# facebookresearch/brainmagick

Measured on AMD Instinct MI355X. Metric: segments/s, 208-ch x 360-sample SimpleConv + ClipLoss training step, higher is better.
Workload: dtype f32 (fp32-accurate: operands split into 2 scaled f16 planes, 3 MFMA products, fp32 accumulate; same parity tolerances as exact fp32, see DESIGN.md §2); 1 GPU; cfg2: gwilliams2022-shaped MEG C=208 T=360, F=120 features, 27 subjects, clip_conv SimpleConv (8985590 params) + ClipLoss + Adam; batch_per_gpu=256, global_batch=256, negatives=local, parallelism=dp1, comm=none, rccl_world=1, candidate_gather=none, distinct_batches=8

## Files before the change

### brainmagick_amd/functional.py

```python

import torch

from . import hip_ops as H



ACT_CODES = {"none": H.ACT_NONE, "gelu": H.ACT_GELU, "relu": H.ACT_RELU, "leaky": H.ACT_LEAKY}


def _c(t: torch.Tensor) -> torch.Tensor:
    return t if t.is_contiguous() else t.contiguous()


_arange_cache = {}


def _arange_i32(n: int, device, repeat: int = 1) -> torch.Tensor:
    key = (n, repeat, device.type, device.index)
    t = _arange_cache.get(key)
    if t is None:
        if len(_arange_cache) > 64:
            _arange_cache.clear()
        t = torch.arange(n, dtype=torch.int32, device=device)
        if repeat != 1:
# ... 49 lines not shown
    if ctx.needs_input_grad[1]:
        if pad is None:
            dw = _conv_weight_grads(dy, x, weight, KS, dil, transposed)
        else:
            a, xl = (x, dy) if transposed else (dy, x)
            dw = H.conv_strided_wgrad(a, xl, KS, stride, dil, pad, out=H.grad_destination(weight)).view(weight.shape)
    dx = None
    if ctx.needs_input_grad[0]:
        if pad is not None:
            wp = H.pack_strided_rows_first(weight) if transposed else H.pack_strided_rows_second(weight)
            _, dx, _ = H.conv_strided(dy, wp, Cin, T, KS, stride, dil, pad, not transposed)
        else:
            if transposed:
                M = weight.shape[1]
                wp = H.pack_weights(weight, 1, Cin, M, 1, 0, M, 1, 0, shape=(T, dil))
            else:
                wp = H.pack_conv_dgrad(weight, (T, dil))
            _, dx, _ = H.conv_nn(dy, wp, Cin, KS, dil, res=res, publish_amax=publish_amax)
    return dx, dw


class Conv1dFn(torch.autograd.Function):

    @staticmethod
    def forward(ctx, x, weight, bias, dil: int, act: int, leak: float, transposed_weight: bool, stride: int = 1,
                pad=None):
        x, weight = _c(x), _c(weight)
        geom = (dil, transposed_weight, stride, pad)
        need_pre = act != H.ACT_NONE and any(ctx.needs_input_grad[:3])
        if need_pre and pad is None:
            pre, _, _ = _layer_forward(x, weight, geom, bias=bias, want_pre=True, want_out=False)
            out = H.affine_act_res(pre, None, None, None, act, leak)
        else:
            pre, out, _ = _layer_forward(x, weight, geom, bias=bias, act=act, leak=leak, want_pre=need_pre)
        ctx.save_for_backward(x, weight, pre)
        ctx.cfg = (geom, act, leak, bias is not None)
        return out

    @staticmethod
    def backward(ctx, dout):
        x, weight, pre = ctx.saved_tensors
        geom, act, leak, has_bias = ctx.cfg
        dout = _c(dout)
        dbias = None
        if act != H.ACT_NONE:
            dy, _, _, dbias = H.act_bn_bwd(dout, pre, None, None, None, None, False, act, leak,
                                           want_dbias=has_bias)
        else:
            dy = dout
            if has_bias:
                dbias = H.channel_sum(dy)
        dx, dw = _layer_backward(ctx, dy, x, weight, geom)
        return (dx, dw, dbias) + (None,) * 6


class ConvBNActFn(torch.autograd.Function):

    @staticmethod
    def forward(ctx, x, weight, bias, gamma, beta, running_mean, running_var, num_batches,
                training: bool, dil: int, act: int, leak: float, residual: bool, momentum: float,
                eps: float, stride: int = 1, pad=None, transposed: bool = False):
        x, weight = _c(x), _c(weight)
        geom = (dil, transposed, stride, pad)
        res = x if residual else None
        needs_grad = any(ctx.needs_input_grad[:5])
        if training:
            pre, _, stats = _layer_forward(x, weight, geom, bias=bias, want_pre=True, want_out=False, want_stats=True)
            mean, invstd, scale, shift = H.bn_finalize(stats, pre.shape[0] * pre.shape[2], gamma, beta, running_mean,
                                                       running_var, num_batches, momentum, eps)
            out = H.affine_act_res(pre, scale, shift, res, act, leak)
        else:
            mean, invstd, scale, shift = H.bn_eval_affine(gamma, beta, running_mean, running_var, eps)
            pre, out, _ = _layer_forward(x, weight, geom, res=res, bias=bias, scale=scale, shift=shift, act=act,
                                         leak=leak, want_pre=needs_grad)
        ctx.save_for_backward(x, weight, pre, scale, shift, mean, invstd)
        ctx.cfg = (geom, training, act, leak, residual, bias is not None)
        return out

    @staticmethod
    def backward(ctx, dout):
        x, weight, pre, scale, shift, mean, invstd = ctx.saved_tensors
        geom, training, act, leak, residual, has_bias = ctx.cfg
        dout = _c(dout)
        dy, dgamma, dbeta, dbias = H.act_bn_bwd(dout, pre, scale, shift, mean, invstd, training, act,
                                                leak, want_affine_grads=True, want_dbias=has_bias)
        dx, dw = _layer_backward(ctx, dy, x, weight, geom, res=dout if residual else None, publish_amax=False)
        return (dx, dw, dbias, dgamma, dbeta) + (None,) * 13


class GLUConvFn(torch.autograd.Function):

    @staticmethod
    def forward(ctx, x, weight, bias):
        x, weight = _c(x), _c(weight)
        M, Cin, KS = weight.shape
        u, _, _ = H.conv_nn(x, H.pack_conv_fwd(weight, (x.shape[2], 1)), M, KS, 1, bias=bias, want_pre=True,
                            want_out=False)
        out = H.glu_fwd(u)
        ctx.save_for_backward(x, weight, u)
        ctx.has_bias = bias is not None
        return out

    @staticmethod
    def backward(ctx, dout):
        x, weight, u = ctx.saved_tensors
        M, Cin, KS = weight.shape
# ... 404 lines not shown
```

### brainmagick_amd/hip_ops.py

```python
import ctypes
import typing as tp

import numpy as np
import torch

from ._lib import lib, check, BmHipError

ACT_NONE, ACT_GELU, ACT_RELU, ACT_LEAKY = 0, 1, 2, 3
BKC = 16

import os as _os
DEFAULT_COMPUTE_DTYPE = "f16x2"
COMPUTE_DTYPES = ("f32", "f32x3", "f16x2")
_compute_dtype = _os.environ.get("BM_COMPUTE_DTYPE", DEFAULT_COMPUTE_DTYPE)
if _compute_dtype not in COMPUTE_DTYPES:
    raise ValueError(f"BM_COMPUTE_DTYPE must be one of {COMPUTE_DTYPES}, got {_compute_dtype!r}")


def set_compute_dtype(name: str):
    global _compute_dtype
    if name not in COMPUTE_DTYPES:
        raise ValueError(f"compute dtype must be one of {COMPUTE_DTYPES}, got {name!r}")
    _compute_dtype = name

# ... 208 lines not shown
        e["used"] = _weights_epoch
        if e["stamp"] != (_weights_epoch, src._version):
            self.refresh()
        return e["dst"]

    def refresh(self):
        global pack_launches
        stale = [k for k, e in self.entries.items()
                 if e["used"] < _weights_epoch - self.KEEP or e["src"].data_ptr() != e["ptr"]]
        for k in stale:
            del self.entries[k]
        if stale:
            self.table = None
        ents = list(self.entries.values())
        if not ents:
            return
        if self.table is None:
            nb = lib().bm_pack_h2_job_bytes()
            host = ctypes.create_string_buffer(nb * len(ents))
            block0 = 0
            for i, e in enumerate(ents):
                n = lib().bm_pack_h2_job_fill(ctypes.c_void_p(ctypes.addressof(host) + i * nb), _p(e["src"]),
                                              _p(e["dst"]), *e["geom"], None, block0)
                if n < 0:
                    raise BmHipError("bm_pack_h2_job_fill: bad arguments %r" % (e["geom"],))
                block0 += n
            self.table = torch.frombuffer(bytearray(host.raw), dtype=torch.uint8).to(self.device)
            self.total_blocks = block0
        max_nk = max(e["geom"][2] * e["geom"][3] for e in ents)
        check(lib().bm_pack_weights_h2_batch(_p(self.table), len(ents), self.total_blocks, max_nk, _stream()),
              "bm_pack_weights_h2_batch")
        pack_launches += 1
        for e in ents:
            e["stamp"] = (_weights_epoch, e["src"]._version)


_pack_plans: tp.Dict[tp.Tuple[str, int], _PackPlan] = {}


def _pack_plan(device) -> _PackPlan:
    key = (device.type, device.index if device.index is not None else torch.cuda.current_device())
    if key not in _pack_plans:
        _pack_plans[key] = _PackPlan(torch.device(*key))
    return _pack_plans[key]


def pack_weights(src: torch.Tensor, G: int, M: int, Cin: int, KS: int, sg: int, sm: int, sc: int,
                 sj: int, flip: bool = False, alpha: tp.Optional[torch.Tensor] = None,
                 shape: tp.Optional[tp.Tuple[int, int]] = None) -> torch.Tensor:
    _req(src, "pack_weights.src")
    mode = _compute_dtype
    if mode == "f16x2":
        if shape is not None and lib().bm_conv_h2_covers(Cin, M, shape[0], KS, shape[1]):
            if alpha is None and src.requires_grad and src.is_leaf:
                return _pack_plan(src.device).get(src, (G, M, Cin, KS, sg, sm, sc, sj, int(flip)))
            nbytes = lib().bm_packed_weight_bytes_h2(G, M, Cin, KS)
            dst = torch.empty(nbytes, device=src.device, dtype=torch.uint8)
            check(lib().bm_pack_weights_h2(_p(src), _p(dst), G, M, Cin, KS, sg, sm, sc, sj, int(flip),
                                           _p(_opt(alpha, "alpha")), _stream()), "bm_pack_weights_h2")
            global pack_launches
            pack_launches += 1
            dst._bm_mode = "f16x2"
            dst._bm_groups = G
            return dst
        mode = "f32x3"
    if mode == "f32x3":
        n = lib().bm_packed_weight_elems_x3(G, M, Cin, KS)
        dst = torch.empty(n, device=src.device, dtype=torch.bfloat16)
        check(lib().bm_pack_weights_x3(_p(src), _p(dst), G, M, Cin, KS, sg, sm, sc, sj, int(flip),
                                       _p(_opt(alpha, "alpha")), _stream()), "bm_pack_weights_x3")
        dst._bm_mode = mode
        return dst
    return pack_weights_f32(src, M, Cin, KS, sm, sc, sj, G, sg, flip, alpha)


def pack_weights_f32(src: torch.Tensor, M: int, Cin: int, KS: int, sm: int, sc: int, sj: int, G: int = 1, sg: int = 0,
                     flip: bool = False, alpha: tp.Optional[torch.Tensor] = None) -> torch.Tensor:
    _req(src, "pack_weights_f32.src")
    dst = torch.empty(lib().bm_packed_weight_elems(G, M, Cin, KS), device=src.device, dtype=torch.float32)
    check(lib().bm_pack_weights(_p(src), _p(dst), G, M, Cin, KS, sg, sm, sc, sj, int(flip), _p(_opt(alpha, "alpha")),
                                _stream()), "bm_pack_weights")
    return dst


def pack_conv_fwd(weight: torch.Tensor, shape=None) -> torch.Tensor:
    M, Cin, KS = weight.shape
    return pack_weights(weight, 1, M, Cin, KS, 0, Cin * KS, KS, 1, shape=shape)


def pack_conv_dgrad(weight: torch.Tensor, shape=None) -> torch.Tensor:
    M, Cin, KS = weight.shape
    return pack_weights(weight, 1, Cin, M, KS, 0, KS, Cin * KS, 1, flip=True, shape=shape)


def _conv_outputs(x: torch.Tensor, M: int, T: int, want_pre: bool, want_out: bool, stats_shape=None):
    def new(shape, want=True):
        return torch.empty(shape, device=x.device, dtype=torch.float32) if want and shape is not None else None
    return new((x.shape[0], M, T), want_pre), new((x.shape[0], M, T), want_out), new(stats_shape)


def conv_nn(x: torch.Tensor, wpacked: torch.Tensor, M: int, KS: int = 1, dil: int = 1,
            widx: tp.Optional[torch.Tensor] = None, bias=None, scale=None, shift=None, res=None,
            act: int = ACT_NONE, leak: float = 0., want_pre: bool = False, want_out: bool = True,
            want_stats: bool = False, out: tp.Optional[torch.Tensor] = None, bias_gstride: int = 0,
            publish_amax: bool = True):
    _req(x, "conv_nn.x")
    mode = getattr(wpacked, "_bm_mode", "f32")
    _req(wpacked, "conv_nn.w", {"f32": torch.float32, "f16x2": torch.uint8}.get(mode, torch.bfloat16))
    B, Cin, T = x.shape
    channel_major = want_stats and mode == "f16x2"
    stats_shape = None if not want_stats else (M, lib().bm_conv_h2_stats_tiles(B, T), 2) if channel_major else \
        (lib().bm_conv_stats_tiles(B, T), M, 2)
    y_pre, y_out, stats = _conv_outputs(x, M, T, want_pre, want_out and out is None, stats_shape)
    if channel_major:
        stats._bm_channel_major = True
    if out is not None:
        _req(out, "conv_nn.out")
        assert want_out and out.numel() == B * M * T, (out.shape, (B, M, T))
        y_out = _touched(out)
    if res is not None:
        _req(res, "conv_nn.res")
        assert res.shape == (B, M, T), (res.shape, (B, M, T))
    common = (_p(_opt(widx, "widx", torch.int32)), _p(_opt(bias, "bias")), bias_gstride, _p(_opt(scale, "scale")),
              _p(_opt(shift, "shift")), _p(res), M * T, _p(y_pre), _p(y_out), M * T, _p(stats), B, Cin, M, T,
              KS, dil, act, leak)
    if mode == "f16x2":
# ... 287 lines not shown
    _req(stats, "bn_finalize.stats")
    channel_major = getattr(stats, "_bm_channel_major", False)
    (C, ntiles, _) = stats.shape if channel_major else (stats.shape[1], stats.shape[0], 2)
    mean, invstd, scale, shift = (torch.empty(C, device=stats.device, dtype=torch.float32)
                                  for _ in range(4))
    check((lib().bm_bn_finalize_cm if channel_major else lib().bm_bn_finalize)(_p(stats), ntiles, C, count, _p(_opt(gamma, "gamma")),
                               _p(_opt(beta, "beta")), _p(_opt(running_mean, "running_mean")),
                               _p(_opt(running_var, "running_var")),
                               _p(_opt(num_batches, "num_batches", torch.int64)), momentum, eps,
                               _p(mean), _p(invstd), _p(scale), _p(shift), _stream()),
          "bm_bn_finalize")
    return mean, invstd, scale, shift


def bn_eval_affine(gamma, beta, running_mean, running_var, eps: float):
    _req(running_mean, "running_mean")
    C = running_mean.numel()
    mean, invstd, scale, shift = (torch.empty(C, device=running_mean.device, dtype=torch.float32)
                                  for _ in range(4))
    check(lib().bm_bn_eval_affine(C, _p(_opt(gamma, "gamma")), _p(_opt(beta, "beta")),
                                  _p(running_mean), _p(_req(running_var, "running_var")), eps,
                                  _p(mean), _p(invstd), _p(scale), _p(shift), _stream()),
          "bm_bn_eval_affine")
    return mean, invstd, scale, shift


def affine_act_res(y, scale, shift, res, act: int, leak: float = 0.):
    _req(y, "affine_act_res.y")
    B, C, T = y.shape
    out = torch.empty_like(y)
    check(lib().bm_affine_act_res(_p(y), _p(_opt(scale, "scale")), _p(_opt(shift, "shift")),
                                  _p(_opt(res, "res")), _p(out), B, C, T, act, leak, *_slot_args(_amax_slot(out)),
                                  _stream()), "bm_affine_act_res")
    return out


def act_bn_bwd(dout, y, scale, shift, mean, invstd, bn_train: bool, act: int, leak: float = 0.,
               want_affine_grads: bool = False, want_dbias: bool = True):
    _req(dout, "act_bn_bwd.dout")
    _req(y, "act_bn_bwd.y")
    B, C, T = y.shape
    dy = torch.empty_like(y)
    dgamma = torch.empty(C, device=y.device, dtype=torch.float32) if want_affine_grads else None
    dbeta = torch.empty(C, device=y.device, dtype=torch.float32) if want_affine_grads else None
    dbias = torch.empty(C, device=y.device, dtype=torch.float32) if want_dbias else None
    nbytes = lib().bm_act_bn_bwd_workspace_bytes(B, C)
    ws = torch.empty(nbytes, device=y.device, dtype=torch.uint8)
    slot = _amax_slot(dy)
    check(lib().bm_act_bn_bwd(_p(dout), _p(y), _p(_opt(scale, "scale")), _p(_opt(shift, "shift")),
                              _p(_opt(mean, "mean")), _p(_opt(invstd, "invstd")), int(bn_train),
                              _p(dy), _p(dgamma), _p(dbeta), _p(dbias), _p(ws), nbytes, B, C, T, act,
                              leak, *_slot_args(slot), _p(_row_amax_out(dy, slot)), _stream()), "bm_act_bn_bwd")
    return dy, dgamma, dbeta, dbias


def channel_sum(x: torch.Tensor) -> torch.Tensor:
    _req(x, "channel_sum.x")
    B, C, T = x.shape
    out = torch.empty(C, device=x.device, dtype=torch.float32)
    nbytes = lib().bm_channel_sum_workspace_bytes(B, C)
    ws = torch.empty(nbytes, device=x.device, dtype=torch.uint8)
    check(lib().bm_channel_sum(_p(x), C * T, _p(out), _p(ws), nbytes, B, C, T, _stream()),
          "bm_channel_sum")
    return out


def channel_stats(x: torch.Tensor) -> torch.Tensor:
    _req(x, "channel_stats.x")
    B, C, T = x.shape
    stats = torch.empty(lib().bm_channel_stats_splits(B), C, 2, device=x.device, dtype=torch.float32)
    check(lib().bm_channel_stats(_p(x), _p(stats), B, C, T, _stream()), "bm_channel_stats")
    return stats


def time_sums_t(x: torch.Tensor) -> torch.Tensor:
    _req(x, "time_sums_t.x")
    B, C, T = x.shape
    out = torch.empty(C, B, device=x.device, dtype=torch.float32)
    check(lib().bm_time_sums_t(_p(x), _p(out), B, C, T, _stream()), "bm_time_sums_t")
    return out


def glu_fwd(u: torch.Tensor) -> torch.Tensor:
    _req(u, "glu_fwd.u")
    B, C2, T = u.shape
    out = torch.empty(B, C2 // 2, T, device=u.device, dtype=torch.float32)
    check(lib().bm_glu_fwd(_p(u), _p(out), B, C2 // 2, T, *_slot_args(_amax_slot(out)), _stream()), "bm_glu_fwd")
    return out


def glu_bwd(dout: torch.Tensor, u: torch.Tensor, want_dbias: bool = True):
    _req(dout, "glu_bwd.dout")
    _req(u, "glu_bwd.u")
    B, C2, T = u.shape
    H = C2 // 2
    du = torch.empty_like(u)
    dbias = torch.empty(C2, device=u.device, dtype=torch.float32) if want_dbias else None
    nbytes = lib().bm_glu_bwd_workspace_bytes(B, H)
    ws = torch.empty(nbytes, device=u.device, dtype=torch.uint8)
    slot = _amax_slot(du)
    check(lib().bm_glu_bwd(_p(dout), _p(u), _p(du), _p(dbias), _p(ws), nbytes, B, H, T,
                           *_slot_args(slot), _p(_row_amax_out(du, slot)), _stream()), "bm_glu_bwd")
    return du, dbias


def fourier_emb(positions: torch.Tensor, D: int, margin: float = 0.2) -> torch.Tensor:
# ... 783 lines not shown
```

### brainmagick_amd/models/simpleconv.py

```python
import random
import typing as tp

import torch
from torch import nn

from .common import (
    ConvSequence, ScaledEmbedding, SubjectLayers, ChannelMerger, ChannelDropout, DualPathRNN, make_activation)
from .. import functional as BF
from .. import hip_ops as H


_FUSE_FRONT_END = True


class SimpleConv(nn.Module):

    def __init__(self, in_channels: tp.Dict[str, int], out_channels: int, hidden: tp.Dict[str, int],
                 depth: int = 4, concatenate: bool = False, linear_out: bool = False,
                 complex_out: bool = False, kernel_size: int = 5, growth: float = 1.,
                 dilation_growth: int = 2, dilation_period: tp.Optional[int] = None, skip: bool = False,
                 post_skip: bool = False, scale: tp.Optional[float] = None, rewrite: bool = False,
                 groups: int = 1, glu: int = 0, glu_context: int = 0, glu_glu: bool = True,
                 gelu: bool = False, dual_path: int = 0, conv_dropout: float = 0.0,
                 dropout_input: float = 0.0, batch_norm: bool = False, relu_leakiness: float = 0.0,
# ... 110 lines not shown
        if x.dtype != torch.float32:
            raise TypeError(f"SimpleConv expects fp32 inputs like the reference, got {x.dtype}")

        if self.subsampled_meg_channels is not None:
            x = x * self._channel_keep
        if self.dropout is not None:
            x = self.dropout(x, batch)
        fused = self._front_end_is_linear_chain() and _FUSE_FRONT_END
        if fused:
            positions_u, layout_index, ban_center, radius = self.merger.layouts_and_ban(x, batch)
            fused = positions_u.shape[0] * self.subject_layers.weights.shape[0] <= x.shape[0]
        self.front_end_fused = fused
        if fused:
            conv = self.initial_linear[0]
            x = BF.FusedFrontEndFn.apply(x, self.merger.heads, conv.weight, conv.bias, self.subject_layers.weights,
                                         positions_u, layout_index, subjects, ban_center, radius)
        elif self.merger is not None and self._front_end_is_linear_chain() and _FUSE_FRONT_END:
            x = BF.ChannelMergerFn.apply(x, self.merger.heads, positions_u, layout_index, ban_center, radius)
        elif self.merger is not None:
            x = self.merger(x, batch)
        if fused:
            pass
        elif self.initial_linear is not None:
            mods = list(self.initial_linear)
            i = 0
            while i < len(mods):
                conv = mods[i]
                act = mods[i + 1] if i + 1 < len(mods) and not isinstance(mods[i + 1], nn.Conv1d) \
                    else None
                x = BF.Conv1dFn.apply(x, conv.weight, conv.bias, 1,
                                      act.code if act is not None else H.ACT_NONE,
                                      act.leak if act is not None else 0., False)
                i += 2 if act is not None else 1
        if self.subject_layers is not None and not fused:
            x = self.subject_layers(x, subjects)
        if self.subject_embedding is not None:
            emb = self.subject_embedding(subjects)[:, :, None]
            x = torch.cat([x, emb.expand(-1, -1, length)], dim=1)
        inputs["meg"] = x

        if self._concatenate:
            x = self.encoders["concat"](torch.cat([v for _, v in sorted(inputs.items())], dim=1))
        elif len(self.encoders) == 1:
            x = self.encoders["meg"](x)
        else:
            x = torch.cat([self.encoders[name](v) for name, v in sorted(inputs.items())], dim=1)
        if self.dual_path is not None:
            x = self.dual_path(x)
        if self.final is not None:
            if isinstance(self.final, nn.ConvTranspose1d):
                x = BF.Conv1dFn.apply(x, self.final.weight, self.final.bias, 1, H.ACT_NONE, 0., True)
            else:
                conv, act, tconv = self.final[0], self.final[1], self.final[2]
                x = BF.Conv1dFn.apply(x, conv.weight, conv.bias, 1, act.code, act.leak, False)
                x = BF.Conv1dFn.apply(x, tconv.weight, tconv.bias, 1, H.ACT_NONE, 0., True)
        assert x.shape[-1] >= length
        return x if x.shape[-1] == length else x[:, :, :length]
```

### include/bm_hip.h

```cpp
#ifndef BM_HIP_H
#define BM_HIP_H
#ifdef __cplusplus
extern "C" {
#endif

#define BM_ACT_NONE 0
#define BM_ACT_GELU 1
#define BM_ACT_RELU 2
#define BM_ACT_LEAKY 3

int bm_version(void);
const char* bm_last_error(void);
int bm_device_count(void);

int bm_conv_mt_for(int M);
int bm_conv_mpad(int M);
int bm_conv_stats_tiles(int B, int T);
long bm_packed_weight_elems(int G, int M, int Cin, int KS);
int bm_pack_weights(const float* src, float* dst, int G, int M, int Cin, int KS, long sg, long sm,
                    long sc, long sj, int flip, const float* alpha_ptr, void* stream);
int bm_group_by_index(const long* idx, int B, int G, int* order, int* seg, int* err_flag, void* stream);
int bm_index_to_i32(const long* idx, int B, int G, int* out, int* err_flag, void* stream);
int bm_reduce_splits(const float* part, float* out, int G, int nsplit, int M, int Cn, int KS, long sg,
                     long sm, long sc, long sj, void* stream);
// ... 8 lines not shown
int bm_conv_strided_stats_tiles(int B, int Tout, int stride, int transposed);
int bm_conv1d_strided(const float* x, long x_bstride, const float* wpacked, const float* bias,
                      const float* ep_scale, const float* ep_shift, float* y_pre, float* y_out, long y_bstride,
                      float* stats, int B, int Cin, int M, int T, int Tout, int KS, int stride, int dil, int pad,
                      int act, float leak, void* stream);
int bm_conv1d_transposed(const float* x, long x_bstride, const float* wpacked, const float* bias,
                         const float* ep_scale, const float* ep_shift, float* y_pre, float* y_out, long y_bstride,
                         float* stats, int B, int Cin, int M, int T, int Tout, int KS, int stride, int dil, int pad,
                         int act, float leak, void* stream);
int bm_conv1d_strided_wgrad_suggest_splits(int R, int Q, int KS, int S, int U);
int bm_conv1d_strided_wgrad(const float* a, long a_sstride, const float* xl, long xl_sstride, float* part, int S,
                            int R, int Q, int U, int L, int KS, int stride, int dil, int pad, int nsplit,
                            void* stream);

int bm_lstm_layer_fwd(const float* whh0, const float* whh1, const float* gx0, const float* gx1, float* y,
                      float* gates0, float* gates1, float* c0, float* c1, int H, int B, int T, int dirs,
                      void* stream);
int bm_lstm_layer_bwd(const float* whh0, const float* whh1, const float* dy, const float* gates0,
                      const float* gates1, const float* c0, const float* c1, float* dg0, float* dg1,
                      float* dc0, float* dc1, int H, int B, int T, int dirs, void* stream);

long bm_packed_weight_elems_x3(int G, int M, int Cin, int KS);
int bm_pack_weights_x3(const float* src, void* dst, int G, int M, int Cin, int KS, long sg, long sm,
                       long sc, long sj, int flip, const float* alpha_ptr, void* stream);
int bm_conv1d_nn_x3(const float* x, long x_bstride, const void* wpacked, const int* widx,
                    const float* bias, long bias_gstride, const float* ep_scale, const float* ep_shift, const float* res,
                    long res_bstride, float* y_pre, float* y_out, long y_bstride, float* stats, int B,
                    int Cin, int M, int T, int KS, int dil, int act, float leak, void* stream);
int bm_gemm_nt_x3(const float* a, long a_sstride, long a_rstride, const float* x, long x_sstride,
                  long x_rstride, const int* order, const int* seg, float* part, int S, int G, int M,
                  int Cn, int T, int KS, int dil, int nsplit, void* stream);
int bm_conv_x3_mt_for(int M);
int bm_conv_x3_mpad(int M);

int bm_conv_h2_mw_for(int M);
int bm_conv_h2_mpad(int M);
int bm_conv_h2_covers(int Cin, int M, int T, int KS, int dil);
long bm_packed_weight_bytes_h2(int G, int M, int Cin, int KS);
int bm_pack_weights_h2(const float* src, void* dst, int G, int M, int Cin, int KS, long sg, long sm, long sc,
                       long sj, int flip, const float* alpha_ptr, void* stream);
int bm_pack_h2_job_bytes(void);
int bm_pack_h2_job_fill(void* job, const float* src, void* dst, int G, int M, int Cin, int KS, long sg, long sm,
                        long sc, long sj, int flip, const float* alpha_ptr, int block0);
int bm_pack_weights_h2_batch(const void* jobs_dev, int njobs, int total_blocks, int max_nk, void* stream);
int bm_amax_ws_elems(void);
int bm_amax(const float* x, long n, float* out, float* amax_ws, void* stream);
int bm_amax_checked(const float* x, long n, float* out, float* amax_ws, int* nonfinite_flag, void* stream);
int bm_conv_h2_stats_tiles(int B, int T);
int bm_conv1d_nn_h2(const float* x, long x_bstride, const float* x_amax, const void* wpacked, const int* widx,
                    const float* bias, long bias_gstride, const float* ep_scale, const float* ep_shift, const float* res,
                    long res_bstride, float* y_pre, float* y_out, long y_bstride, float* stats, int B, int Cin,
                    int M, int T, int KS, int dil, int act, float leak, int G, float* y_amax_out, float* amax_ws,
                    void* stream);

int bm_gemm_nt_h2_covers(int M, int Cn, int KS, int S, int T, int G, int dil, int ordered);
int bm_gemm_nt_h2_suggest_splits(int M, int Cn, int KS, int S, int T);
int bm_gemm_nt_h2(const float* a, long a_sstride, long a_rstride, const float* a_amax, const float* x,
                  long x_sstride, long x_rstride, const float* x_amax, float* part, int S, int M, int Cn, int T,
                  int KS, int dil, int nsplit, void* stream);
int bm_gemm_nt_h2_rows(const float* a, long a_sstride, long a_rstride, const float* a_amax, const float* a_row_amax,
                       const float* x, long x_sstride, long x_rstride, const float* x_amax, float* part, int S,
                       int M, int Cn, int T, int KS, int dil, int nsplit, void* stream);

int bm_gemm_nt_h2_grouped(const float* a, long a_sstride, long a_rstride, const float* a_amax, const float* x,
                          long x_sstride, long x_rstride, const float* x_amax, const int* order, const int* seg,
                          float* part, int S, int G, int M, int Cn, int T, int nsplit, void* stream);
int bm_gemm_nt_h2_suggest_splits_grouped(int M, int Cn, int KS, int S, int T, int G);

int bm_clip_scores_h2_covers(int B, int Bc, long K);
int bm_clip_scores_h2_suggest_splits(int B, int Bc, long K);
int bm_clip_scores_h2(const float* est, const float* est_amax, const float* cand, const float* cand_amax, float* part,
                      int B, int Bc, long K, int nsplit, void* stream);

int bm_gemm_nt_suggest_splits(int M, int Cn, int KS, int S, int T, int G);
int bm_clip_suggest_splits(int M, int Cn, int S, int T);
int bm_gemm_nt(const float* a, long a_sstride, long a_rstride, const float* x, long x_sstride,
               long x_rstride, const int* order, const int* seg, float* part, int S, int G, int M,
               int Cn, int T, int KS, int dil, int nsplit, void* stream);

int bm_bn_finalize(const float* stats, int ntiles, int C, long count, const float* gamma,
                   const float* beta, float* running_mean, float* running_var, long* num_batches,
                   float momentum, float eps, float* mean, float* invstd, float* scale, float* shift,
                   void* stream);
int bm_bn_finalize_cm(const float* stats, int ntiles, int C, long count, const float* gamma,
                   const float* beta, float* running_mean, float* running_var, long* num_batches,
                   float momentum, float eps, float* mean, float* invstd, float* scale, float* shift,
                   void* stream);
int bm_bn_eval_affine(int C, const float* gamma, const float* beta, const float* running_mean,
                      const float* running_var, float eps, float* mean, float* invstd, float* scale,
                      float* shift, void* stream);
int bm_affine_act_res(const float* y, const float* scale, const float* shift, const float* res,
                      float* out, int B, int C, int T, int act, float leak, float* amax_out, float* amax_ws,
                      void* stream);
int bm_bwd_nsplit(int B);
long bm_act_bn_bwd_workspace_bytes(int B, int C);
int bm_act_bn_bwd_set_fused(int mode);
int bm_act_bn_bwd_set_poll_limit(int polls);
long bm_act_bn_bwd_fused_fallbacks(void);
int bm_act_bn_bwd_fused_covers(int B, int C, int T);
int bm_act_bn_bwd(const float* dout, const float* y, const float* scale, const float* shift,
                  const float* mean, const float* invstd, int bn_train, float* dy, float* dgamma,
                  float* dbeta, float* dbias, void* workspace, long workspace_bytes, int B, int C,
                  int T, int act, float leak, float* amax_out, float* amax_ws, float* amax_rows_out,
                  void* stream);
long bm_channel_sum_workspace_bytes(int B, int C);
int bm_channel_sum(const float* x, long bstride, float* out, void* workspace, long workspace_bytes,
// ... 133 lines not shown
```

Baseline: 17580 segments/s.

## Fuse head activation with second 1x1 conv in dedicated forward and backward kernels

Adds dedicated HIP kernels for the final projection head. The forward applies the activation to the first conv's pre-activation inside the second 1x1 conv's MFMA loop and writes the activated tensor and amax in the same pass. The backward fuses the transposed 1x1 conv with the activation gradient and a per-tile dbias and row-amax reduction, which a small fold kernel then finishes. This removes separate activation, bias-reduction and amax passes over the large hidden tensor, at the cost of specialised code that only covers M≤128 and hidden≤3840.

Result: no change. 17680 segments/s, median of 4 (+0.6%).

```diff
diff --git a/brainmagick_amd/csrc/head_h2.hip b/brainmagick_amd/csrc/head_h2.hip
--- /dev/null
+++ b/brainmagick_amd/csrc/head_h2.hip
@@ -0,0 +1,427 @@
+#include <cstdlib>
+#include "mfma_split.h"
+#include "bm_block.h"
+
+typedef _Float16 f16x8 __attribute__((ext_vector_type(8)));
+
+#define HD_T 128
+#define HD_OOR 0x40000000
+
+extern "C" int bm_conv_h2_mpad(int M);
+extern "C" int bm_amax(const float* x, long n, float* out, float* ws, void* stream);
+
+static int g_head_fused = -1;
+extern "C" int bm_head_set_fused(int mode) {
+    const int prev = g_head_fused;
+    g_head_fused = mode < 0 ? -1 : (mode ? 1 : 0);
+    return prev;
+}
+extern "C" int bm_head_fused_enabled() {
+    if (g_head_fused < 0) {
+        const char* e = getenv("BM_HEAD_FUSED");
+        g_head_fused = (e && e[0] == '0') ? 0 : 1;
+    }
+    return g_head_fused;
+}
+extern "C" int bm_head_h2_covers(int B, int hidden, int M, int T) {
+    if (B <= 0 || hidden <= 0 || M <= 0 || M > HD_T || T <= 0 || T % 4 != 0) return 0;
+    if ((long)hidden * T * 4 >= HD_OOR || (long)B * hidden * T >= 0x7fffffffL) return 0;
+    if ((long)hidden > 3840 || (long)B * cdiv(T, HD_T) > 0x7fffffL) return 0;
+    return 1;
+}
+
+__device__ __forceinline__ f32x4 hd_ld128(__amdgpu_buffer_rsrc_t r, int off) {
+    return __builtin_bit_cast(f32x4, __builtin_amdgcn_raw_buffer_load_b128(r, off, 0, 0));
+}
+__device__ __forceinline__ void hd_mma(f32x16 (&acc)[2][2], const f16x8 (&af)[2][2], const f16x8 (&bf)[2][2]) {
+#pragma unroll
+    for (int term = 0; term < 3; ++term) {
+        const int pa = term == 0 ? 1 : 0, pb = term == 1 ? 1 : 0;
+#pragma unroll
+        for (int mt = 0; mt < 2; ++mt)
+#pragma unroll
+            for (int nt = 0; nt < 2; ++nt)
+                acc[mt][nt] = __builtin_amdgcn_mfma_f32_32x32x16_f16(af[pa][mt], bf[pb][nt], acc[mt][nt], 0, 0, 0);
+    }
+}
+
+struct HeadFwdArgs {
+    const float* pre;
+    float* out;
+    const void* wp;
+    const float* wscale;
+    const float* bias;
+    float* y;
+    const float* pre_amax;
+    BmAmaxDst y_amax, out_amax;
+    int B, C, M, T, nchunk, ntiles_n, act;
+    float leak;
+};
+
+__global__ __launch_bounds__(256, 2) void head_act_conv_h2_kernel(HeadFwdArgs a) {
+    __shared__ __attribute__((aligned(16))) u32x4 Xs[2][2][4][HD_T];
+    __shared__ float rowp[2][HD_T];
+    __shared__ float amax_sh[2][4];
+    const int tid = threadIdx.x, lane = tid & 63;
+    const int wave = __builtin_amdgcn_readfirstlane(tid >> 6);
+    const int wm = wave >> 1, wn = wave & 1, nl = lane & 31, h = lane >> 5;
+    const int ntile = blockIdx.x % a.ntiles_n, b = blockIdx.x / a.ntiles_n;
+    const int n0 = ntile * HD_T;
+    const int C = a.C, T = a.T;
+    float sx, sx_inv;
+    bm_scale_from_amax(bm_amax_load(a.pre_amax), sx, sx_inv);
+    if (tid < HD_T) {
+        rowp[0][tid] = a.wscale[tid] * sx_inv;
+        rowp[1][tid] = (a.bias && tid < a.M) ? a.bias[tid] : 0.f;
+    }
+    const __amdgpu_buffer_rsrc_t xr = bm_buffer_rsrc(a.pre + (long)b * C * T, (unsigned)(C * T * 4));
+    const __amdgpu_buffer_rsrc_t wr = bm_buffer_rsrc(a.wp, (unsigned)(a.nchunk * 8 * HD_T * 16));
+    const int q = tid & 31, r = tid >> 5;
+    const int t0 = n0 + 4 * q;
+    const bool colok = t0 < T;
+    const int xoff = colok ? (4 * r * T + t0) * 4 : HD_OOR;
+    const int crow = T * 4;
+    float* outp = a.out ? a.out + (long)b * C * T + (long)(4 * r) * T + t0 : nullptr;
+    const int wvoff = (h * HD_T + wm * 64 + nl) * 16;
+
+    f32x16 acc[2][2];
+#pragma unroll
+    for (int i = 0; i < 2; ++i)
+#pragma unroll
+        for (int k = 0; k < 2; ++k)
+#pragma unroll
+            for (int e = 0; e < 16; ++e) acc[i][k][e] = 0.f;
+
+    f32x4 xc[4], xn[4];
+#pragma unroll
+    for (int j = 0; j < 4; ++j) xc[j] = hd_ld128(xr, xoff + j * crow);
+    float amx_out = 0.f;
+    for (int i = 0; i < a.nchunk; ++i) {
+#pragma unroll
+        for (int j = 0; j < 4; ++j) xn[j] = hd_ld128(xr, xoff + ((i + 1) * 32 + j) * crow);
+        f16x8 af[2][2][2];
+#pragma unroll
+        for (int ks = 0; ks < 2; ++ks)
+#pragma unroll
+            for (int p = 0; p < 2; ++p)
+#pragma unroll
+                for (int mt = 0; mt < 2; ++mt)
+                    af[ks][p][mt] = __builtin_bit_cast(f16x8, __builtin_amdgcn_raw_buffer_load_b128(
+                        wr, wvoff + mt * 512, ((i * 8 + p * 4 + 2 * ks) * HD_T) * 16, 0));
+        float z[4][4];
+#pragma unroll
+        for (int j = 0; j < 4; ++j) {
+#pragma unroll
+            for (int e = 0; e < 4; ++e) {
+                z[j][e] = bm_act(xc[j][e] * 1.f + 0.f, a.act, a.leak);
+                amx_out = fmaxf(amx_out, fabsf(z[j][e]));
+            }
+            if (outp && colok && i * 32 + 4 * r + j < C)
+                *reinterpret_cast<f32x4*>(outp + (long)(i * 32 + j) * T) = f32x4{z[j][0], z[j][1], z[j][2], z[j][3]};
+        }
+        char* xw = reinterpret_cast<char*>(&Xs[i & 1][0][r >> 1][4 * q]) + (r & 1) * 8;
+#pragma unroll
+        for (int e = 0; e < 4; ++e) {
+            unsigned h0, l0, h1, l1;
+            bm_split_pair(z[0][e], z[1][e], sx, h0, l0);
+            bm_split_pair(z[2][e], z[3][e], sx, h1, l1);
+            *reinterpret_cast<uint2*>(xw + e * 16) = make_uint2(h0, h1);
+            *reinterpret_cast<uint2*>(xw + e * 16 + sizeof(Xs[0][0])) = make_uint2(l0, l1);
+        }
+        __syncthreads();
+#pragma unroll
+        for (int ks = 0; ks < 2; ++ks) {
+            f16x8 bf[2][2];
+#pragma unroll
+            for (int p = 0; p < 2; ++p)
+#pragma unroll
+                for (int nt = 0; nt < 2; ++nt)
+                    bf[p][nt] = __builtin_bit_cast(f16x8, Xs[i & 1][p][2 * ks + h][wn * 64 + nt * 32 + nl]);
+            hd_mma(acc, af[ks], bf);
+        }
+#pragma unroll
+        for (int j = 0; j < 4; ++j) xc[j] = xn[j];
+    }
+
+    float amx = 0.f;
+    float* yb = a.y + (long)b * a.M * T;
+#pragma unroll
+    for (int mt = 0; mt < 2; ++mt)
+#pragma unroll
+        for (int e = 0; e < 16; ++e) {
+            const int row = wm * 64 + mt * 32 + (e & 3) + 8 * (e >> 2) + 4 * h;
+            const float f = rowp[0][row], bb = rowp[1][row];
+#pragma unroll
+            for (int nt = 0; nt < 2; ++nt) {
+                const int col = n0 + wn * 64 + nt * 32 + nl;
+                const float v = fmaf(acc[mt][nt][e], f, bb);
+                if (row < a.M && col < T) {
+                    amx = fmaxf(amx, fabsf(v));
+                    yb[row * T + col] = v;
+                }
+            }
+        }
+    bm_publish_amax(amx, a.y_amax, amax_sh[0]);
+    bm_publish_amax(amx_out, a.out_amax, amax_sh[1]);
+}
+
+static bool hd_aligned16(const void* p, const void* q = nullptr, const void* r = nullptr) {
+    return (((uintptr_t)p | (uintptr_t)q | (uintptr_t)r) & 15) == 0;
+}
+
+extern "C" int bm_head_act_conv_h2(const float* pre, const float* pre_amax, const void* wpacked, const float* bias,
+                                   float* out, float* y, int B, int C, int M, int T, int act, float leak,
+                                   float* y_amax_out, float* out_amax_out, float* amax_ws, void* stream) {
+    BM_REQUIRE(pre && pre_amax && wpacked && y, "head_act_conv_h2: null pointer");
+    BM_REQUIRE(bm_head_h2_covers(B, C, M, T), "head_act_conv_h2: shape not covered (B=%d C=%d M=%d T=%d)", B, C, M, T);
+    BM_REQUIRE(hd_aligned16(pre, out, wpacked) && ((uintptr_t)y & 3) == 0, "head_act_conv_h2: pre / out / weights must be 16-byte aligned");
+    BM_REQUIRE(bm_conv_h2_mpad(M) == HD_T, "head_act_conv_h2: packed rows");
+    BM_REQUIRE(!(y_amax_out || out_amax_out) || amax_ws, "head_act_conv_h2: the maxima need the amax workspace");
+    HeadFwdArgs a;
+    a.pre = pre; a.out = out; a.wp = wpacked; a.bias = bias; a.y = y; a.pre_amax = pre_amax;
+    a.B = B; a.C = C; a.M = M; a.T = T; a.act = act; a.leak = leak;
+    a.nchunk = cdiv(C, 32);
+    a.ntiles_n = cdiv(T, HD_T);
+    a.wscale = reinterpret_cast<const float*>(reinterpret_cast<const char*>(wpacked) + (long)a.nchunk * 2 * 4 * HD_T * 8 * 2);
+    if (!out) out_amax_out = nullptr;
+    const int nblocks = B * a.ntiles_n;
+    const bool publish = 2L * nblocks <= BM_AMAX_WS;
+    a.y_amax = BmAmaxDst{publish && y_amax_out ? amax_ws : nullptr};
+    a.out_amax = BmAmaxDst{publish && out_amax_out ? amax_ws + nblocks : nullptr};
+    hipStream_t s = (hipStream_t)stream;
+    hipLaunchKernelGGL(head_act_conv_h2_kernel, dim3((unsigned)nblocks), dim3(256), 0, s, a);
+    if (int rc = bm_check_launch("head_act_conv_h2")) return rc;
+    if (publish) {
+        if (int rc = bm_amax_done(a.y_amax, nblocks, y_amax_out, s)) return rc;
+        return bm_amax_done(a.out_amax, nblocks, out_amax_out, s);
+    }
+    if (y_amax_out)
+        if (int rc = bm_amax(y, (long)B * M * T, y_amax_out, amax_ws, stream)) return rc;
+    if (out_amax_out) return bm_amax(out, (long)B * C * T, out_amax_out, amax_ws, stream);
+    return BM_OK;
+}
+
+struct HeadBwdArgs {
+    const float* dy;
+    const float* pre;
+    const void* wp;
+    const float* wscale;
+    float* dpre;
+    const float* dy_amax;
+    float2* part;
+    int B, C, M, T, Mpad, nk, ntiles_n, act;
+    float leak;
+};
+
+__global__ __launch_bounds__(256, 2) void head_conv_dact_h2_kernel(HeadBwdArgs a) {
+    extern __shared__ __attribute__((aligned(16))) unsigned char hd_smem[];
+    __shared__ float rowf[HD_T];
+    __shared__ float2 red[2][HD_T];
+    u32x4* Ys = reinterpret_cast<u32x4*>(hd_smem);
+    const int tid = threadIdx.x, lane = tid & 63;
+    const int wave = __builtin_amdgcn_readfirstlane(tid >> 6);
+    const int wm = wave >> 1, wn = wave & 1, nl = lane & 31, h = lane >> 5;
+    const int C = a.C, T = a.T, M = a.M, nk = a.nk;
+    const int nrc = (C + HD_T - 1) / HD_T;
+    const int Cp = nrc * HD_T;
+    const int id = bm_xcd_remap(blockIdx.x, gridDim.x);
+    const int rc = id % nrc, tile = id / nrc;
+    const int ntile = tile % a.ntiles_n, b = tile / a.ntiles_n;
+    const int n0 = ntile * HD_T;
+    const int pstride = nk * 4 * HD_T;
+    float sy, sy_inv;
+    bm_scale_from_amax(bm_amax_load(a.dy_amax), sy, sy_inv);
+
+    const __amdgpu_buffer_rsrc_t wr = bm_buffer_rsrc(a.wp, (unsigned)((long)nk * 8 * a.Mpad * 16));
+    const __amdgpu_buffer_rsrc_t pr = bm_buffer_rsrc(a.pre + (long)b * C * T, (unsigned)(C * T * 4));
+    const int col0 = n0 + wn * 64 + nl;
+    const bool cok[2] = {col0 < T, col0 + 32 < T};
+    const int rbase = rc * HD_T + wm * 64;
+    float pv[2][2][16];
+#pragma unroll
+    for (int mt = 0; mt < 2; ++mt)
+#pragma unroll
+        for (int nt = 0; nt < 2; ++nt)
+#pragma unroll
+            for (int e = 0; e < 16; ++e) {
+                const int row = rbase + mt * 32 + (e & 3) + 8 * (e >> 2) + 4 * h;
+                const int off = cok[nt] ? (row * T + col0 + nt * 32) * 4 : HD_OOR;
+                pv[mt][nt][e] = __builtin_bit_cast(float, __builtin_amdgcn_raw_buffer_load_b32(pr, off, 0, 0));
+            }
+    int arow[2];
+#pragma unroll
+    for (int mt = 0; mt < 2; ++mt) arow[mt] = min(rbase + mt * 32 + nl, a.Mpad - 1) * 16;
+    f16x8 af0[2][2], af1[2][2];
+#define HD_LOAD_A(AF_, K16_)                                                                              \
+    _Pragma("unroll") for (int p = 0; p < 2; ++p)                                                         \
+        _Pragma("unroll") for (int mt = 0; mt < 2; ++mt)                                                  \
+            AF_[p][mt] = __builtin_bit_cast(f16x8, __builtin_amdgcn_raw_buffer_load_b128(                 \
+                wr, ((((K16_) >> 1) * 8 + ((K16_) & 1) * 2 + h) + p * 4) * a.Mpad * 16 + arow[mt], 0, 0));
+    HD_LOAD_A(af0, 0)
+
+    {
+        const __amdgpu_buffer_rsrc_t yr = bm_buffer_rsrc(a.dy + (long)b * M * T, (unsigned)(M * T * 4));
+        const int q = tid & 31, r = tid >> 5;
+        const int t0 = n0 + 4 * q;
+        const int yoff = t0 < T ? (4 * r * T + t0) * 4 : HD_OOR;
+        f32x4 v[4][4];
+#pragma unroll
+        for (int p = 0; p < 4; ++p)
+            if (p < nk)
+#pragma unroll
+                for (int j = 0; j < 4; ++j) v[p][j] = hd_ld128(yr, yoff + (p * 32 + j) * T * 4);
+#pragma unroll
+        for (int p = 0; p < 4; ++p)
+            if (p < nk) {
+                char* yw = reinterpret_cast<char*>(Ys + (p * 4 + (r >> 1)) * HD_T + 4 * q) + (r & 1) * 8;
+#pragma unroll
+                for (int e = 0; e < 4; ++e) {
+                    unsigned h0, l0, h1, l1;
+                    bm_split_pair(v[p][0][e], v[p][1][e], sy, h0, l0);
+                    bm_split_pair(v[p][2][e], v[p][3][e], sy, h1, l1);
+                    *reinterpret_cast<uint2*>(yw + e * 16) = make_uint2(h0, h1);
+                    *reinterpret_cast<uint2*>(yw + e * 16 + pstride * 16) = make_uint2(l0, l1);
+                }
+            }
+        if (tid < HD_T) rowf[tid] = a.wscale[min(rc * HD_T + tid, a.Mpad - 1)] * sy_inv;
+    }
+    __syncthreads();
+
+    float* db = a.dpre + (long)b * C * T;
+    const u32x4* yrd = Ys + h * HD_T + wn * 64 + nl;
+    const int act = a.act == BM_ACT_GELU ? BM_ACT_GELU_FASTGRAD : a.act;
+    const bool b4 = lane & 16, b3 = lane & 8, b2 = lane & 4, b1 = lane & 2;
+    f32x16 acc[2][2];
+#pragma unroll
+    for (int i = 0; i < 2; ++i)
+#pragma unroll
+        for (int k = 0; k < 2; ++k)
+#pragma unroll
+            for (int e = 0; e < 16; ++e) acc[i][k][e] = 0.f;
+    for (int c32 = 0; c32 < nk; ++c32) {
+        f16x8 bf[2][2];
+        HD_LOAD_A(af1, 2 * c32 + 1)
+#pragma unroll
+        for (int p = 0; p < 2; ++p)
+#pragma unroll
+            for (int nt = 0; nt < 2; ++nt)
+                bf[p][nt] = __builtin_bit_cast(f16x8, yrd[p * pstride + (4 * c32) * HD_T + nt * 32]);
+        hd_mma(acc, af0, bf);
+        HD_LOAD_A(af0, min(2 * c32 + 2, 2 * nk - 1))
+#pragma unroll
+        for (int p = 0; p < 2; ++p)
+#pragma unroll
+            for (int nt = 0; nt < 2; ++nt)
+                bf[p][nt] = __builtin_bit_cast(f16x8, yrd[p * pstride + (4 * c32 + 2) * HD_T + nt * 32]);
+        hd_mma(acc, af1, bf);
+    }
+#undef HD_LOAD_A
+    {
+        const float* fl = rowf + wm * 64 + 4 * h;
+#pragma unroll
+        for (int mt = 0; mt < 2; ++mt) {
+            float s1[16], mx[16];
+#pragma unroll
+            for (int e = 0; e < 16; ++e) {
+                const int dr = mt * 32 + (e & 3) + 8 * (e >> 2);
+                const int row = rbase + dr + 4 * h;
+                const float f = fl[dr];
+                float g[2];
+#pragma unroll
+                for (int nt = 0; nt < 2; ++nt) {
+                    g[nt] = (acc[mt][nt][e] * f) * bm_act_grad(pv[mt][nt][e], act, a.leak);
+                    if (row < C && cok[nt]) db[row * T + col0 + nt * 32] = g[nt];
+                    else g[nt] = 0.f;
+                }
+                s1[e] = g[0] + g[1];
+                mx[e] = fmaxf(fabsf(g[0]), fabsf(g[1]));
+            }
+#define HD_FOLD(N_, BIT_, MASK_)                                                                  \
+            _Pragma("unroll") for (int i = 0; i < N_; ++i) {                                      \
+                const float k1 = BIT_ ? s1[i + N_] : s1[i], g1 = BIT_ ? s1[i] : s1[i + N_];        \
+                const float k2 = BIT_ ? mx[i + N_] : mx[i], g2 = BIT_ ? mx[i] : mx[i + N_];        \
+                s1[i] = k1 + __shfl_xor(g1, MASK_);                                               \
+                mx[i] = fmaxf(k2, __shfl_xor(g2, MASK_));                                         \
+            }
+            HD_FOLD(8, b4, 16)
+            HD_FOLD(4, b3, 8)
+            HD_FOLD(2, b2, 4)
+            HD_FOLD(1, b1, 2)
+#undef HD_FOLD
+            s1[0] += __shfl_xor(s1[0], 1);
+            mx[0] = fmaxf(mx[0], __shfl_xor(mx[0], 1));
+            const int e = (b4 ? 8 : 0) + (b3 ? 4 : 0) + (b2 ? 2 : 0) + (b1 ? 1 : 0);
+            if (!(lane & 1)) red[wn][wm * 64 + mt * 32 + (e & 3) + 8 * (e >> 2) + 4 * h] = float2{s1[0], mx[0]};
+        }
+        __syncthreads();
+        if (tid < HD_T) {
+            const float2 u = red[0][tid], w = red[1][tid];
+            a.part[(long)tile * Cp + rc * HD_T + tid] = float2{u.x + w.x, fmaxf(u.y, w.y)};
+        }
+    }
+}
+
+__global__ __launch_bounds__(256) void head_fold_rows_kernel(const float2* __restrict__ part, int ntiles, int Cp,
+                                                             float* __restrict__ dbias, float* __restrict__ rowmax) {
+    __shared__ double ssum[4];
+    __shared__ float smax[4];
+    const int c = blockIdx.x;
+    double s = 0.0;
+    float m = 0.f;
+    for (int t = threadIdx.x; t < ntiles; t += 256) {
+        const float2 p = part[(long)t * Cp + c];
+        s += (double)p.x;
+        m = fmaxf(m, p.y);
+    }
+    s = bm_block_sum<4>(s, ssum);
+    m = bm_block_max<4>(m, smax);
+    if (threadIdx.x == 0) {
+        if (dbias) dbias[c] = (float)s;
+        rowmax[c] = m;
+    }
+}
+
+extern "C" long bm_head_conv_dact_workspace_bytes(int B, int C, int T) {
+    return (long)B * cdiv(T, HD_T) * cdiv(C, HD_T) * HD_T * (long)sizeof(float2);
+}
+
+extern "C" int bm_head_conv_dact_h2(const float* dy, const float* dy_amax, const float* pre, const void* wpacked,
+                                    float* dpre, float* dbias, void* workspace, long workspace_bytes, int B, int C,
+                                    int M, int T, int act, float leak, float* amax_out, float* amax_ws,
+                                    float* amax_rows_out, void* stream) {
+    BM_REQUIRE(dy && dy_amax && pre && wpacked && dpre && workspace, "head_conv_dact_h2: null pointer");
+    BM_REQUIRE(bm_head_h2_covers(B, C, M, T), "head_conv_dact_h2: shape not covered (B=%d C=%d M=%d T=%d)", B, C, M, T);
+    BM_REQUIRE(hd_aligned16(dy, wpacked) && (((uintptr_t)pre | (uintptr_t)dpre) & 3) == 0,
+               "head_conv_dact_h2: dy / weights must be 16-byte aligned");
+    BM_REQUIRE(!amax_out || amax_ws, "head_conv_dact_h2: amax_out needs the amax workspace");
+    BM_REQUIRE(C <= BM_AMAX_WS, "head_conv_dact_h2: too many channels for the amax workspace");
+    if (workspace_bytes < bm_head_conv_dact_workspace_bytes(B, C, T))
+        return bm_set_error(BM_ERR_WORKSPACE, "head_conv_dact_h2: workspace too small");
+    HeadBwdArgs a;
+    a.dy = dy; a.pre = pre; a.wp = wpacked; a.dpre = dpre; a.dy_amax = dy_amax; a.part = (float2*)workspace;
+    a.B = B; a.C = C; a.M = M; a.T = T; a.act = act; a.leak = leak;
+    a.Mpad = bm_conv_h2_mpad(C);
+    a.nk = cdiv(M, 32);
+    a.ntiles_n = cdiv(T, HD_T);
+    a.wscale = reinterpret_cast<const float*>(reinterpret_cast<const char*>(wpacked) + (long)a.nk * 2 * 4 * a.Mpad * 8 * 2);
+    const int ntiles = B * a.ntiles_n;
+    const int nblocks = ntiles * cdiv(C, HD_T);
+    const size_t lds = (size_t)a.nk * 2 * 4 * HD_T * 16;
+    static bool attr_set = false;
+    if (!attr_set) {
+        hipError_t e = hipFuncSetAttribute(reinterpret_cast<const void*>(head_conv_dact_h2_kernel),
+                                           hipFuncAttributeMaxDynamicSharedMemorySize, 4 * 2 * 4 * HD_T * 16);
+        if (e != hipSuccess) return bm_set_error((int)e, "head_conv_dact_h2: hipFuncSetAttribute: %s", hipGetErrorString(e));
+        attr_set = true;
+    }
+    hipStream_t s = (hipStream_t)stream;
+    hipLaunchKernelGGL(head_conv_dact_h2_kernel, dim3((unsigned)nblocks), dim3(256), lds, s, a);
+    if (int rc = bm_check_launch("head_conv_dact_h2")) return rc;
+    if (!dbias && !amax_out) return BM_OK;
+    float* rowmax = amax_rows_out && amax_out ? amax_rows_out : amax_ws;
+    BM_REQUIRE(rowmax, "head_conv_dact_h2: dbias needs the amax workspace");
+    hipLaunchKernelGGL(head_fold_rows_kernel, dim3((unsigned)C), dim3(256), 0, s, a.part, ntiles, cdiv(C, HD_T) * HD_T,
+                       dbias, rowmax);
+    if (int rc = bm_check_launch("head_fold_rows")) return rc;
+    return amax_out ? bm_amax_finalize(rowmax, C, amax_out, s) : BM_OK;
+}
diff --git a/brainmagick_amd/functional.py b/brainmagick_amd/functional.py
--- a/brainmagick_amd/functional.py
+++ b/brainmagick_amd/functional.py
@@ -125,6 +125,45 @@
                 dbias = H.channel_sum(dy)
         dx, dw = _layer_backward(ctx, dy, x, weight, geom)
         return (dx, dw, dbias) + (None,) * 6
+
+
+class HeadFn(torch.autograd.Function):
+
+    @staticmethod
+    def forward(ctx, x, w1, b1, w2, b2, act: int, leak: float):
+        x, w1, w2 = _c(x), _c(w1), _c(w2)
+        geom1 = (1, False, 1, None)
+        _, pre, _ = _layer_forward(x, w1, geom1, bias=b1)
+        y, out = H.head_act_conv(pre, w2, b2, act, leak, want_out=ctx.needs_input_grad[3])
+        ctx.save_for_backward(x, w1, w2, pre, out)
+        ctx.cfg = (geom1, act, leak, b1 is not None, b2 is not None)
+        return y
+
+    @staticmethod
+    def backward(ctx, dy):
+        x, w1, w2, pre, out = ctx.saved_tensors
+        geom1, act, leak, has_b1, has_b2 = ctx.cfg
+        dy = _c(dy)
+        hidden, M = w2.shape[0], w2.shape[1]
+        db2 = H.channel_sum(dy) if has_b2 else None
+        dw2 = _conv_weight_grads(dy, out, w2, 1, 1, True) if ctx.needs_input_grad[3] else None
+        dx = dw1 = db1 = None
+        if any(ctx.needs_input_grad[:3]):
+            if dy.data_ptr() % 16 == 0:
+                dpre, db1 = H.head_conv_dact(dy, pre, w2, act, leak, want_dbias=has_b1)
+            else:
+                wp = H.pack_weights(w2, 1, hidden, M, 1, 0, M, 1, 0, shape=(dy.shape[2], 1))
+                _, dh, _ = H.conv_nn(dy, wp, hidden, 1, 1)
+                dpre, _, _, db1 = H.act_bn_bwd(dh, pre, None, None, None, None, False, act, leak, want_dbias=has_b1)
+            dx, dw1 = _layer_backward(ctx, dpre, x, w1, geom1)
+        return dx, dw1, db1, dw2, db2, None, None
+
+
+def head(x, w1, b1, w2, b2, act: int, leak: float):
+    if act != H.ACT_NONE and abs(leak) <= 1. and H.head_fused_covers(x, w1, w2):
+        return HeadFn.apply(x, w1, b1, w2, b2, act, leak)
+    x = Conv1dFn.apply(x, w1, b1, 1, act, leak, False)
+    return Conv1dFn.apply(x, w2, b2, 1, H.ACT_NONE, 0., True)
 
 
 class ConvBNActFn(torch.autograd.Function):
diff --git a/brainmagick_amd/hip_ops.py b/brainmagick_amd/hip_ops.py
--- a/brainmagick_amd/hip_ops.py
+++ b/brainmagick_amd/hip_ops.py
@@ -284,17 +284,7 @@
     mode = _compute_dtype
     if mode == "f16x2":
         if shape is not None and lib().bm_conv_h2_covers(Cin, M, shape[0], KS, shape[1]):
-            if alpha is None and src.requires_grad and src.is_leaf:
-                return _pack_plan(src.device).get(src, (G, M, Cin, KS, sg, sm, sc, sj, int(flip)))
-            nbytes = lib().bm_packed_weight_bytes_h2(G, M, Cin, KS)
-            dst = torch.empty(nbytes, device=src.device, dtype=torch.uint8)
-            check(lib().bm_pack_weights_h2(_p(src), _p(dst), G, M, Cin, KS, sg, sm, sc, sj, int(flip),
-                                           _p(_opt(alpha, "alpha")), _stream()), "bm_pack_weights_h2")
-            global pack_launches
-            pack_launches += 1
-            dst._bm_mode = "f16x2"
-            dst._bm_groups = G
-            return dst
+            return pack_weights_h2(src, G, M, Cin, KS, sg, sm, sc, sj, flip, alpha)
         mode = "f32x3"
     if mode == "f32x3":
         n = lib().bm_packed_weight_elems_x3(G, M, Cin, KS)
@@ -304,6 +294,22 @@
         dst._bm_mode = mode
         return dst
     return pack_weights_f32(src, M, Cin, KS, sm, sc, sj, G, sg, flip, alpha)
+
+
+def pack_weights_h2(src: torch.Tensor, G: int, M: int, Cin: int, KS: int, sg: int, sm: int, sc: int, sj: int,
+                    flip: bool = False, alpha: tp.Optional[torch.Tensor] = None) -> torch.Tensor:
+    global pack_launches
+    _req(src, "pack_weights_h2.src")
+    if alpha is None and src.requires_grad and src.is_leaf:
+        return _pack_plan(src.device).get(src, (G, M, Cin, KS, sg, sm, sc, sj, int(flip)))
+    nbytes = lib().bm_packed_weight_bytes_h2(G, M, Cin, KS)
+    dst = torch.empty(nbytes, device=src.device, dtype=torch.uint8)
+    check(lib().bm_pack_weights_h2(_p(src), _p(dst), G, M, Cin, KS, sg, sm, sc, sj, int(flip),
+                                   _p(_opt(alpha, "alpha")), _stream()), "bm_pack_weights_h2")
+    pack_launches += 1
+    dst._bm_mode = "f16x2"
+    dst._bm_groups = G
+    return dst
 
 
 def pack_weights_f32(src: torch.Tensor, M: int, Cin: int, KS: int, sm: int, sc: int, sj: int, G: int = 1, sg: int = 0,
@@ -697,6 +703,94 @@
                               _p(dy), _p(dgamma), _p(dbeta), _p(dbias), _p(ws), nbytes, B, C, T, act,
                               leak, *_slot_args(slot), _p(_row_amax_out(dy, slot)), _stream()), "bm_act_bn_bwd")
     return dy, dgamma, dbeta, dbias
+
+
+def set_head_fused(on: tp.Optional[bool]) -> None:
+    lib().bm_head_set_fused(-1 if on is None else int(bool(on)))
+
+
+def head_fused_covers(x: torch.Tensor, w1: torch.Tensor, w2: torch.Tensor) -> bool:
+    if _compute_dtype != "f16x2" or not lib().bm_head_fused_enabled():
+        return False
+    if x.dim() != 3 or w1.dim() != 3 or w2.dim() != 3 or w1.shape[2] != 1 or w2.shape[2] != 1:
+        return False
+    B, Cin, T = x.shape
+    hidden, M = w2.shape[0], w2.shape[1]
+    if w1.shape[0] != hidden or w1.shape[1] != Cin or not all(t.is_cuda and t.dtype == torch.float32 for t in (x, w1, w2)):
+        return False
+    if not lib().bm_head_h2_covers(B, hidden, M, T) or not lib().bm_conv_h2_covers(Cin, hidden, T, 1, 1):
+        return False
+    return x.is_contiguous() and x.data_ptr() % 16 == 0
+
+
+def _head_out(t, shape, name):
+    if t is None:
+        return None
+    _req(t, name)
+    assert tuple(t.shape) == tuple(shape), (name, t.shape, shape)
+    return t
+
+
+def head_act_conv(pre: torch.Tensor, w2: torch.Tensor, bias, act: int, leak: float = 0., want_out: bool = True,
+                  y: tp.Optional[torch.Tensor] = None, out: tp.Optional[torch.Tensor] = None):
+    _req(pre, "head_act_conv.pre")
+    _req(w2, "head_act_conv.w2")
+    B, C, T = pre.shape
+    M = w2.shape[1]
+    assert w2.shape[0] == C and w2.shape[2] == 1, (w2.shape, C)
+    wp = pack_weights_h2(w2, 1, M, C, 1, 0, 1, M, 0)
+    pre_amax = amax(pre)
+    y = _head_out(y, (B, M, T), "head_act_conv.y")
+    out = _head_out(out, (B, C, T), "head_act_conv.out") if want_out else None
+    if y is not None:
+        _touched(y)
+    if out is not None:
+        _touched(out)
+    if y is None:
+        y = torch.empty(B, M, T, device=pre.device, dtype=torch.float32)
+    if want_out and out is None:
+        out = torch.empty_like(pre)
+    y_slot = _amax_slot(y)
+    out_slot = _amax_slot(out) if out is not None else None
+
+    def launch():
+        check(lib().bm_head_act_conv_h2(_p(pre), _p(pre_amax), _p(wp), _p(_opt(bias, "bias")), _p(out), _p(y), B, C, M, T,
+                                        act, leak, _p(y_slot), _p(out_slot), _p(_stream_ws("amax", pre.device)),
+                                        _stream()), "bm_head_act_conv_h2")
+    _timed("conv_nn_h2w_kernel<1,2,act>", 2.0 * B * T * M * C, launch)
+    return y, out
+
+
+def head_conv_dact(dy: torch.Tensor, pre: torch.Tensor, w2: torch.Tensor, act: int, leak: float = 0.,
+                   want_dbias: bool = True, dpre: tp.Optional[torch.Tensor] = None,
+                   dbias: tp.Optional[torch.Tensor] = None):
+    _req(dy, "head_conv_dact.dy")
+    _req(pre, "head_conv_dact.pre")
+    _req(w2, "head_conv_dact.w2")
+    B, C, T = pre.shape
+    M = w2.shape[1]
+    assert w2.shape[0] == C and w2.shape[2] == 1 and dy.shape == (B, M, T), (w2.shape, dy.shape, pre.shape)
+    wp = pack_weights_h2(w2, 1, C, M, 1, 0, M, 1, 0)
+    dy_amax = amax(dy)
+    dpre = _head_out(dpre, (B, C, T), "head_conv_dact.dpre")
+    if dpre is not None:
+        _touched(dpre)
+    if dpre is None:
+        dpre = torch.empty_like(pre)
+    dbias = _head_out(dbias, (C,), "head_conv_dact.dbias") if want_dbias else None
+    if want_dbias and dbias is None:
+        dbias = torch.empty(C, device=pre.device, dtype=torch.float32)
+    nbytes = lib().bm_head_conv_dact_workspace_bytes(B, C, T)
+    ws = torch.empty(nbytes, device=pre.device, dtype=torch.uint8)
+    slot = _amax_slot(dpre)
+    rows = _row_amax_out(dpre, slot)
+
+    def launch():
+        check(lib().bm_head_conv_dact_h2(_p(dy), _p(dy_amax), _p(pre), _p(wp), _p(dpre), _p(dbias), _p(ws), nbytes, B, C,
+                                         M, T, act, leak, _p(slot), _p(_stream_ws("amax", pre.device)), _p(rows),
+                                         _stream()), "bm_head_conv_dact_h2")
+    _timed("conv_nn_h2w_kernel<1,2,dact>", 2.0 * B * T * M * C, launch)
+    return dpre, dbias
 
 
 def channel_sum(x: torch.Tensor) -> torch.Tensor:
diff --git a/brainmagick_amd/models/simpleconv.py b/brainmagick_amd/models/simpleconv.py
--- a/brainmagick_amd/models/simpleconv.py
+++ b/brainmagick_amd/models/simpleconv.py
@@ -186,7 +186,6 @@
                 x = BF.Conv1dFn.apply(x, self.final.weight, self.final.bias, 1, H.ACT_NONE, 0., True)
             else:
                 conv, act, tconv = self.final[0], self.final[1], self.final[2]
-                x = BF.Conv1dFn.apply(x, conv.weight, conv.bias, 1, act.code, act.leak, False)
-                x = BF.Conv1dFn.apply(x, tconv.weight, tconv.bias, 1, H.ACT_NONE, 0., True)
+                x = BF.head(x, conv.weight, conv.bias, tconv.weight, tconv.bias, act.code, act.leak)
         assert x.shape[-1] >= length
         return x if x.shape[-1] == length else x[:, :, :length]
diff --git a/include/bm_hip.h b/include/bm_hip.h
--- a/include/bm_hip.h
+++ b/include/bm_hip.h
@@ -84,6 +84,17 @@
                     long res_bstride, float* y_pre, float* y_out, long y_bstride, float* stats, int B, int Cin,
                     int M, int T, int KS, int dil, int act, float leak, int G, float* y_amax_out, float* amax_ws,
                     void* stream);
+
+int bm_head_set_fused(int mode);
+int bm_head_fused_enabled(void);
+int bm_head_h2_covers(int B, int hidden, int M, int T);
+int bm_head_act_conv_h2(const float* pre, const float* pre_amax, const void* wpacked, const float* bias, float* out,
+                        float* y, int B, int C, int M, int T, int act, float leak, float* y_amax_out,
+                        float* out_amax_out, float* amax_ws, void* stream);
+long bm_head_conv_dact_workspace_bytes(int B, int C, int T);
+int bm_head_conv_dact_h2(const float* dy, const float* dy_amax, const float* pre, const void* wpacked, float* dpre,
+                         float* dbias, void* workspace, long workspace_bytes, int B, int C, int M, int T, int act,
+                         float leak, float* amax_out, float* amax_ws, float* amax_rows_out, void* stream);
 
 int bm_gemm_nt_h2_covers(int M, int Cn, int KS, int S, int T, int G, int dil, int ordered);
 int bm_gemm_nt_h2_suggest_splits(int M, int Cn, int KS, int S, int T);
```
